# jurihock/sdft

Hardware: AMD Instinct MI355X
Metric: Msamples/s analysis+synthesis, m=1024 Hann fp64; achieved HBM GB/s vs peak (higher is better)
Workload: dtype f64

## Files before the change

sdft_amd/csrc/sdft_capi.inc:

```

#include "sdft_plan.hpp"

#pragma clang fp contract(off)

#define SDFT_CAT_(a, b) a##b
#define SDFT_CAT(a, b) SDFT_CAT_(a, b)
#define SDFT_FN(name) SDFT_CAT(SDFT_CAT(sdft_hip_, name), SDFT_CAT(_, SDFT_SUFFIX))

namespace {
using plan_t = sdfthip::Plan<SDFT_TD, SDFT_FD>;
using fdx_t = sdfthip::cx<SDFT_FD>;
inline plan_t* P(void* p) { return static_cast<plan_t*>(p); }
inline const plan_t* P(const void* p) { return static_cast<const plan_t*>(p); }
}

extern "C" {

void* SDFT_FN(alloc_batch)(size_t dftsize, int window, double latency, size_t channels)
{
  plan_t* p = new (std::nothrow) plan_t();
  if (!p) { sdfthip::set_error("sdft_alloc", "out of host memory"); return nullptr; }
  if (!p->create(dftsize, window, latency, channels)) { p->destroy(); delete p; return nullptr; }
  return p;
}
// ... 146 lines not shown
  if (!p || !key) return -1;
  plan_t* q = P(p);
  if (!strcmp(key, "async")) { if (!value) (void)q->pipe_join(); q->async = value != 0; }
  else if (!strcmp(key, "pipeline")) { if (!value) (void)q->pipe_join(); q->opt_pipeline = value; }
  else if (!strcmp(key, "carry")) q->carry_mode = (value || (sizeof(SDFT_FD) == 4 && !q->opt_float_parallel)) ? sdfthip::CARRY_EXACT : sdfthip::CARRY_FAST;
  else if (!strcmp(key, "float_carry_parallel"))
  {
    q->opt_float_parallel = value != 0;
    if (sizeof(SDFT_FD) == 4) q->carry_mode = value ? sdfthip::CARRY_FAST : sdfthip::CARRY_EXACT;
  }
  else if (!strcmp(key, "exact_inverse")) q->opt_exact_inverse = value;
  else if (!strcmp(key, "host_copy")) q->io.opt_host_copy = value;
  else if (!strcmp(key, "host_register")) { q->io.opt_host_register = value; if (!value) q->io.forget_host_buffers(); }
  else if (!strcmp(key, "copy_threads")) { if (value != q->io.opt_copy_threads) q->io.pool.stop(); q->io.opt_copy_threads = value; }
  else if (!strcmp(key, "pinned_io")) q->opt_pinned_io = value;
  else if (!strcmp(key, "spin")) q->opt_spin = value;
  else if (!strcmp(key, "profile")) q->profile = (int)value;
  else if (!strcmp(key, "resident")) { if (!value) (void)q->resident_retire(); q->opt_resident = value; }
  else if (!strcmp(key, "chunk")) q->opt_chunk = value;
  else if (!strcmp(key, "segments")) q->opt_segments = value;
  else if (!strcmp(key, "chain")) q->opt_chain = value;
  else if (!strcmp(key, "self_carry")) q->opt_self = value;
  else if (!strcmp(key, "hop_kernel")) q->opt_hop_kernel = value;
  else if (!strcmp(key, "fused_exact")) q->opt_fused_exact = value;
  else if (!strcmp(key, "inverse_rows")) q->opt_inverse_rows = value;
  else if (!strcmp(key, "inverse_tune")) { q->opt_inverse_tune = value; for (auto& t : q->inv_tunes) t.reset_all(); }
  else if (!strcmp(key, "pointers")) q->opt_pointers = value;
  else if (!strcmp(key, "stage_bytes")) q->stage_bytes = value > 0 ? (size_t)value : q->stage_bytes;
#ifdef SDFT_HIP_TEST_HOOKS
  else if (!strcmp(key, "interior")) q->opt_interior = value;
  else if (!strcmp(key, "inverse_verify")) q->opt_inverse_verify = value != 0;
  else if (!strcmp(key, "rows_kernel")) q->opt_rows_kernel = value;
  else if (!strcmp(key, "row_slots_max")) q->opt_row_slots_max = value;
  else if (!strcmp(key, "fft_carry")) q->opt_fft_carry = value;
  else if (!strcmp(key, "fused")) q->opt_fused = value;
  else if (!strcmp(key, "fold")) q->opt_fold = value;
  else if (!strcmp(key, "rows_f32")) q->opt_rows_f32 = value;
  else if (!strcmp(key, "hop_parts")) q->opt_hop_parts = value;
  else if (!strcmp(key, "xcd_map")) q->opt_xcd_map = value;
  else if (!strcmp(key, "chain_block")) q->opt_chain_L = value;
  else if (!strcmp(key, "chain_debug")) q->opt_chain_debug = value;
  else if (!strcmp(key, "relay_waves")) q->opt_relay_waves = value;
  else if (!strcmp(key, "relay_flow")) q->opt_relay_flow = value;
  else if (!strcmp(key, "relay_groups")) q->opt_relay_groups = value;
  else if (!strcmp(key, "inverse_nt")) q->opt_inverse_nt = value;
  else if (!strcmp(key, "inverse_nt_skip_mb")) q->opt_inverse_nt_skip_mb = value;
  else if (!strcmp(key, "inverse_step")) q->opt_inverse_step = value;
  else if (!strcmp(key, "inverse_ordered")) q->opt_inverse_ordered = value;
  else if (!strcmp(key, "host_direct")) q->io.opt_host_direct = value;
  else if (!strcmp(key, "copy_streams")) q->io.opt_copy_streams = value;
  else if (!strcmp(key, "array_group")) q->opt_array_group = value;
  else if (!strcmp(key, "mix_group")) q->opt_mix_group = value;
  else if (!strcmp(key, "mix_block")) q->opt_mix_block = value;
  else if (!strcmp(key, "prefix_cells")) q->opt_prefix_cells = value;
#ifdef SDFT_SELF_STAMPS
  else if (!strcmp(key, "self_stamps")) q->opt_self_stamps = value;
#endif
#endif
  else return -1;
  return 0;
}
long SDFT_FN(get_option)(const void* p, const char* key)
{
  if (!p || !key) return -1;
  const plan_t* q = P(p);
  if (!strcmp(key, "async")) return q->async;
  if (!strcmp(key, "pipeline")) return q->opt_pipeline;
  if (!strcmp(key, "last_pipelined")) return q->last_pipelined;
  if (!strcmp(key, "pipelined_calls")) return (long)q->pipe_calls;
  if (!strcmp(key, "pipelined_ordered")) return (long)q->pipe_ordered;
  if (!strcmp(key, "pipelined_inverse_calls")) return (long)q->inv_calls;
  if (!strcmp(key, "last_inverse_pipelined")) return q->last_inverse_pipelined;
  if (!strcmp(key, "pipeline_streams")) return q->pipe_stream_kind * 10 + q->pipe_stream_attempts;
  if (!strcmp(key, "carry")) return q->carry_mode;
  if (!strcmp(key, "float_carry_parallel")) return q->opt_float_parallel;
  if (!strcmp(key, "ordered_walks")) return q->ordered_walks();
  if (!strcmp(key, "inverse_verify")) return q->opt_inverse_verify;
  if (!strcmp(key, "last_inverse_form")) return q->last_inverse_form;
  if (!strcmp(key, "chunk")) return q->opt_chunk;
  if (!strcmp(key, "interior")) return q->interior_lanes();
  if (!strcmp(key, "tiles")) return q->tiles();
  if (!strcmp(key, "bins_per_lane")) return plan_t::bins_per_lane();
  if (!strcmp(key, "last_chunks")) return q->last_chunks;
  if (!strcmp(key, "last_chunk_len")) return q->last_chunk_len;
  if (!strcmp(key, "cursor")) return (long)q->cursor;
  if (!strcmp(key, "last_kernel")) return q->last_kernel;
  if (!strcmp(key, "rows_kernel")) return q->opt_rows_kernel;
  if (!strcmp(key, "fused")) return q->opt_fused;
  if (!strcmp(key, "last_fused")) return q->last_fused;
  if (!strcmp(key, "last_segments")) return q->last_segments;
  if (!strcmp(key, "last_filterbank_launches")) return q->last_filterbank_launches;
  if (!strcmp(key, "row_slots")) return q->row_slots();
  if (!strcmp(key, "device")) return q->device;
  if (!strcmp(key, "last_chain")) return q->last_chain;
  if (!strcmp(key, "last_fused_exact")) return q->last_fused_exact;
  if (!strcmp(key, "last_fused_fold")) return q->last_fused_fold;
  if (!strcmp(key, "last_process_path")) return q->last_process_path;
  if (!strcmp(key, "fused_exact")) return q->opt_fused_exact;
  if (!strcmp(key, "chain")) return q->opt_chain;
  if (!strcmp(key, "fold")) return q->opt_fold;
  if (!strcmp(key, "last_hop_pipe")) return q->last_hop_pipe;
  if (!strcmp(key, "spin")) return q->opt_spin;
  if (!strcmp(key, "inverse_step")) return q->opt_inverse_step;
  if (!strcmp(key, "inverse_ordered")) return q->opt_inverse_ordered;
  if (!strcmp(key, "inverse_nt_skip_mb")) return q->opt_inverse_nt_skip_mb;
  if (!strcmp(key, "last_inverse_nt")) return q->last_inverse_nt;
  if (!strcmp(key, "last_inverse_skip")) return q->last_inverse_skip;
  if (!strcmp(key, "hop_parts")) return q->opt_hop_parts;
  if (!strcmp(key, "xcd_map")) return q->opt_xcd_map;
  if (!strcmp(key, "inverse_tune")) return q->opt_inverse_tune;
  if (!strcmp(key, "last_inverse_tuned")) return q->last_inverse_tuned;
  if (!strcmp(key, "last_hop_parts")) return q->last_hop_parts;
  if (!strcmp(key, "self_carry")) return q->opt_self;
  if (!strcmp(key, "last_self")) return q->last_self;
  if (!strcmp(key, "last_prefix")) return q->last_prefix;
#ifdef SDFT_HIP_TEST_HOOKS
  if (!strcmp(key, "prefix_cells")) return q->opt_prefix_cells;
#endif
  if (!strcmp(key, "array_group")) return q->array_group();
  if (!strcmp(key, "mix_group")) return q->mix_group_size();
  if (!strcmp(key, "mix_block")) return q->mix_block_size();
  if (!strcmp(key, "host_register")) return q->io.opt_host_register;
  if (!strcmp(key, "host_register_hits")) return q->io.host_reg_hits;
  if (!strcmp(key, "host_copy")) return q->io.opt_host_copy;
  if (!strcmp(key, "copy_threads")) return q->io.opt_copy_threads;
  if (!strcmp(key, "copy_streams")) return q->io.opt_copy_streams;
  if (!strcmp(key, "copy_workers")) return (long)q->io.pool.workers();
  if (!strcmp(key, "host_copies_staged")) return q->io.pin_copies;
  if (!strcmp(key, "host_copy_memcpy_us")) return (long)q->io.pin_us_memcpy;
  if (!strcmp(key, "host_copy_device_us")) return (long)q->io.pin_us_device;
  if (!strcmp(key, "host_register_misses")) return q->io.host_reg_misses;
  if (!strcmp(key, "last_flow")) return q->last_flow;
  if (!strcmp(key, "flag_fallbacks")) return q->flag_fallbacks;
  if (!strcmp(key, "ring_recoveries")) return q->ring_recoveries;
  if (!strcmp(key, "rows_f32")) return q->opt_rows_f32;
  if (!strcmp(key, "last_rows_f32")) return q->last_rows_f32;
  if (!strcmp(key, "resident")) return q->opt_resident;
  if (!strcmp(key, "resident_calls")) return (long)q->res.calls;
  if (!strcmp(key, "resident_launches")) return (long)q->res.launches;
  if (!strcmp(key, "resident_missed")) return (long)q->res.missed;
  if (!strcmp(key, "resident_alive")) return q->res.alive ? 1 : 0;
  if (!strcmp(key, "test_hooks"))
  {
#ifdef SDFT_HIP_TEST_HOOKS
    return 1;
#else
    return 0;
#endif
  }
  return -1;
}
int SDFT_FN(get_profile)(void* p, double* ms, long* calls)
{
  if (!p) return -1;
  plan_t* q = P(p);
  if (!q->synchronize()) return -1;
  for (int s = 0; s < sdfthip::ST_COUNT; ++s)
  {
    if (ms) ms[s] = q->prof_ms[s];
    if (calls) calls[s] = q->prof_calls[s];
    q->prof_ms[s] = 0; q->prof_calls[s] = 0;
  }
  return 0;
}
int SDFT_FN(chain_stats)(void* p, unsigned long long* out32) { return p && P(p)->chain_stats(out32) ? 0 : -1; }
int SDFT_FN(relay_stamps)(void* p, unsigned long long* out, size_t count) { return p && P(p)->relay_stamps(out, count) ? 0 : -1; }
int SDFT_FN(get_state)(void* p, void* acc, void* fid, SDFT_TD* hist, size_t* cursor)
{
  return p && P(p)->get_state(static_cast<fdx_t*>(acc), static_cast<fdx_t*>(fid), hist, cursor) ? 0 : -1;
}
// ... 17 lines not shown
```

sdft_amd/csrc/sdft_forward.hpp:

```cpp

#pragma once

#include "sdft_carry_exact.hpp"

#pragma clang fp contract(off)

namespace sdfthip {

template <typename FD, int WIN> SDFT_D cx<FD> window_tap(cx<FD> m2, cx<FD> m1, cx<FD> c0, cx<FD> p1, cx<FD> p2, FD w)
{
  if constexpr (WIN == WIN_HANN)
  {
    const cx<FD> a = cadd(c0, c0);
    const cx<FD> b = cadd(m1, p1);
    return cscale(csub(a, b), w);
  }
  else if constexpr (WIN == WIN_HAMMING)
  {
    const cx<FD> a = cscale(c0, (FD)(0.54));
    const cx<FD> b = cscale(cadd(m1, p1), (FD)(0.23));
    return cscale(csub(a, b), w);
  }
  else if constexpr (WIN == WIN_BLACKMAN)
  {
// ... 85 lines not shown
  r = block - q * d;
  if (r >= d) { --q; r += d; }
}
template <typename FD> SDFT_D void flow_position(const ForwardArgs<FD>& a, unsigned& chunk, size_t& ch, unsigned block)
{
  unsigned q, r;
  if (a.ready) { uniform_divmod(block, a.ready_channels, a.inv_channels, q, r); chunk = a.chunk0 + q; ch = r; }
  else
  {
    if (a.xcd_map) block = xcd_contiguous(block, a.xcd_map);
    uniform_divmod(block, a.launch_chunks, a.inv_chunks, q, r);
    chunk = a.chunk0 + r; ch = q;
  }
}
template <typename FD> SDFT_D void flow_position(const ForwardArgs<FD>& a, unsigned& chunk, size_t& ch) { flow_position(a, chunk, ch, blockIdx.x); }
constexpr unsigned kFlowPollCap = 1u << 19;
template <typename FD> SDFT_D bool flow_wait(const ForwardArgs<FD>& a, unsigned chunk, size_t ch)
{
  if (!a.ready) return true;
  const unsigned* row = a.ready + (ch * a.chunks + chunk) * (size_t)a.ready_n;
  for (unsigned polls = 0;; ++polls)
  {
    bool ok = true;
    for (unsigned i = threadIdx.x; i < a.ready_n; i += blockDim.x)
      ok = ok && __hip_atomic_load(row + i, __ATOMIC_RELAXED, __HIP_MEMORY_SCOPE_AGENT) == a.ready_seq;
    if (__syncthreads_and(ok ? 1 : 0)) break;
    if (polls > kFlowPollCap)
    {
      if (threadIdx.x == 0 && a.ready_status) __hip_atomic_fetch_add(a.ready_status, 1u, __ATOMIC_RELAXED, __HIP_MEMORY_SCOPE_SYSTEM);
      return false;
    }
    if ((polls & 1023u) == 1023u && a.ready_status)
    {
      const bool gone = threadIdx.x == 0 && __hip_atomic_load(a.ready_status, __ATOMIC_RELAXED, __HIP_MEMORY_SCOPE_SYSTEM) != a.ready_status_seen;
      if (__syncthreads_or(gone ? 1 : 0)) return false;
    }
    __builtin_amdgcn_s_sleep(32);
  }
  __builtin_amdgcn_fence(__ATOMIC_ACQUIRE, "agent");
  asm volatile("s_waitcnt vmcnt(0)" ::: "memory");
  __syncthreads();
  return true;
}

template <typename TD, typename FD> struct SelfArgs
{
  const TD* x;
  size_t x_stride;
  const TD* hist_in;
  TD* hist_out;
  const cx<FD>* acc_in;
  unsigned log2m;
  unsigned lds_deltas;
  const FD* prefix;
#ifdef SDFT_SELF_STAMPS
  unsigned long long* stamps;
#endif
  RadixList rl;
};

template <int CP, int QB, typename TD, typename FD>
SDFT_D void self_fold(const SelfArgs<TD, FD>& sa, cx<FD>* cells, unsigned m, unsigned cursor0, size_t ch, size_t t0)
{
  const TD* xs = sa.x + ch * sa.x_stride;
  const TD* hs = sa.hist_in + ch * (size_t)m;
  const unsigned nthr = blockDim.x;
  const size_t rows = (t0 + m - 1) / m;
  for (unsigned v0 = threadIdx.x; v0 < m; v0 += CP * nthr)
  {
    size_t tv[CP]; FD sum[CP]; TD prev[CP];
#pragma unroll
    for (int c = 0; c < CP; ++c)
    {
      const unsigned v = v0 + (unsigned)c * nthr;
      tv[c] = (size_t)(((v < m ? v : v0) + m - cursor0) % m);
      sum[c] = (FD)0;
      prev[c] = hs[tv[c]];
    }
    for (size_t q = 0; q < rows; q += QB)
    {
      TD cur[CP][QB];
#pragma unroll
      for (int c = 0; c < CP; ++c)
#pragma unroll
        for (int qq = 0; qq < QB; ++qq)
        {
          const size_t t = tv[c] + (q + qq) * (size_t)m;
          cur[c][qq] = xs[t < t0 ? t : t0 - 1];
        }
#pragma unroll
      for (int c = 0; c < CP; ++c)
#pragma unroll
        for (int qq = 0; qq < QB; ++qq)
        {
          const size_t t = tv[c] + (q + qq) * (size_t)m;
          if (t < t0) { const TD dd = cur[c][qq] - prev[c]; sum[c] += (FD)dd; prev[c] = cur[c][qq]; }
        }
    }
#pragma unroll
    for (int c = 0; c < CP; ++c)
    {
      const unsigned v = v0 + (unsigned)c * nthr;
      if (v < m) cells[v] = cmake<FD>(sum[c], (FD)0);
    }
  }
}

template <typename FD>
SDFT_D void lds_fft_dif(cx<FD>* x, unsigned log2m, const cx<FD>* __restrict__ w)
{
  const unsigned m = 1u << log2m;
  unsigned st = 0;
  for (; st + 2 <= log2m; st += 2)
  {
    const unsigned half = m >> (st + 1), quarter = half >> 1;
    for (unsigned i = threadIdx.x; i < (m >> 2); i += blockDim.x)
    {
      const unsigned pos = i & (quarter - 1);
      const unsigned base = ((i - pos) << 2) + pos;
      const cx<FD> a0 = x[base], a1 = x[base + quarter], a2 = x[base + half], a3 = x[base + half + quarter];
      const cx<FD> w1 = w[(size_t)pos << st];
      const cx<FD> w2 = w[(size_t)pos << (st + 1)];
      const cx<FD> b0 = cadd(a0, a2), b2 = cmul(csub(a0, a2), w1);
      const cx<FD> b1 = cadd(a1, a3), tq = cmul(csub(a1, a3), w1);
      const cx<FD> b3 = cmake<FD>(tq.im, -tq.re);
      x[base] = cadd(b0, b1);
      x[base + quarter] = cmul(csub(b0, b1), w2);
      x[base + half] = cadd(b2, b3);
      x[base + half + quarter] = cmul(csub(b2, b3), w2);
    }
    __syncthreads();
  }
  if (st < log2m)
  {
    for (unsigned i = threadIdx.x; i < (m >> 1); i += blockDim.x)
    {
      const cx<FD> p = x[2 * i], q = x[2 * i + 1];
      x[2 * i] = cadd(p, q);
      x[2 * i + 1] = csub(p, q);
    }
    __syncthreads();
  }
}

template <typename FD>
SDFT_D cx<FD>* lds_fft_mixed(cx<FD>* x, unsigned m, const RadixList& rl, const cx<FD>* __restrict__ w)
{
  cx<FD>* y = x + m;
  unsigned ns = 1;
  for (unsigned st = 0; st < rl.count; ++st)
  {
    const unsigned r = rl.r[st];
    const unsigned nr = m / r;
    const unsigned tstep = m / (ns * r);
    const unsigned rstep = nr;
    for (unsigned i = threadIdx.x; i < nr; i += blockDim.x)
    {
      const unsigned k = i % ns;
      cx<FD> v[5];
#pragma unroll
      for (unsigned t = 0; t < 5; ++t)
        if (t < r)
        {
          const cx<FD> in = x[i + t * nr];
          v[t] = t == 0 ? in : cmul(in, w[(size_t)(((unsigned long long)t * k * tstep) % m)]);
        }
      const unsigned base = (i / ns) * ns * r + k;
#pragma unroll
      for (unsigned q = 0; q < 5; ++q)
        if (q < r)
        {
          cx<FD> o = v[0];
#pragma unroll
          for (unsigned t = 1; t < 5; ++t)
            if (t < r) o = cadd(o, cmul(v[t], w[(size_t)(((unsigned long long)q * t * rstep) % m)]));
          y[base + q * ns] = o;
        }
    }
    __syncthreads();
    cx<FD>* tmp = x; x = y; y = tmp;
    ns *= r;
  }
  return x;
}

template <typename TD, typename FD> SDFT_D unsigned self_slot(const SelfArgs<TD, FD>& sa, unsigned k)
{
  return sa.log2m ? (__brev(k) >> (32u - sa.log2m)) : k;
}
template <int CP, int QB, typename TD, typename FD>
SDFT_D cx<FD>* self_carry(const SelfArgs<TD, FD>& sa, const ForwardArgs<FD>& a, cx<FD>* cells, unsigned chunk, size_t ch, size_t t0)
{
  const unsigned m = 2u * a.nbins;
  if (chunk + 1 == a.chunks && sa.hist_out)
  {
    const TD* xv = sa.x + ch * sa.x_stride;
    const TD* hv = sa.hist_in + ch * (size_t)m;
    TD* ho = sa.hist_out + ch * (size_t)m;
    for (size_t i = threadIdx.x; i < m; i += blockDim.x)
    {
      const size_t q = a.n + i;
      ho[i] = (q >= m) ? xv[q - m] : hv[q];
    }
  }
  if (t0 == 0) return nullptr;
#ifdef SDFT_SELF_STAMPS
  const bool st_on = sa.stamps && chunk + 1 == a.chunks && threadIdx.x == 0;
  if (st_on) sa.stamps[1] = __builtin_readcyclecounter();
#endif
  if (sa.prefix)
  {
    const FD* pc = sa.prefix + (ch * a.chunks + chunk) * (size_t)m;
    for (unsigned v = threadIdx.x; v < m; v += blockDim.x) cells[v] = cmake<FD>(pc[v], (FD)0);
  }
  else self_fold<CP, QB>(sa, cells, m, a.cursor0, ch, t0);
  __syncthreads();
#ifdef SDFT_SELF_STAMPS
  if (st_on) sa.stamps[2] = __builtin_readcyclecounter();
#endif
  if (sa.log2m)
  {
    lds_fft_dif(cells, sa.log2m, a.wtab);
#ifdef SDFT_SELF_STAMPS
    if (st_on) sa.stamps[3] = __builtin_readcyclecounter();
#endif
    return cells;
  }
  return lds_fft_mixed(cells, m, sa.rl, a.wtab);
}

template <int G, typename TD, typename FD>
SDFT_D void self_deltas(FD (&dl)[G], const SDFT_CONSTANT TD* xs, const SDFT_CONSTANT TD* hs, size_t tt, size_t span)
{
  TD cur[G], old[G];
#pragma unroll
  for (int u = 0; u < G; ++u) cur[u] = xs[tt + u];
  if (tt + G <= span)
  {
#pragma unroll
    for (int u = 0; u < G; ++u) old[u] = hs[tt + u];
  }
  else if (tt >= span)
  {
#pragma unroll
    for (int u = 0; u < G; ++u) old[u] = xs[tt - span + u];
  }
  else
  {
#pragma unroll
    for (int u = 0; u < G; ++u) old[u] = (tt + u < span) ? hs[tt + u] : xs[tt + u - span];
  }
#pragma unroll
  for (int u = 0; u < G; ++u) { const TD dd = cur[u] - old[u]; dl[u] = (FD)dd; }
}
template <typename TD, typename FD>
SDFT_D FD self_delta1(const SDFT_CONSTANT TD* xs, const SDFT_CONSTANT TD* hs, size_t tt, size_t span)
{
  const TD cur = xs[tt];
  const TD old = (tt < span) ? hs[tt] : xs[tt - span];
  const TD dd = cur - old;
  return (FD)dd;
}

typedef double sdft_v2f64 __attribute__((ext_vector_type(2)));
typedef float sdft_v4f32 __attribute__((ext_vector_type(4)));
typedef float sdft_v2f32 __attribute__((ext_vector_type(2)));
template <typename FD, int BPL> struct StoreVec;
template <> struct StoreVec<double, 1> { using type = sdft_v2f64; };
template <> struct StoreVec<float, 2>  { using type = sdft_v4f32; };
template <> struct StoreVec<float, 1>  { using type = sdft_v2f32; };

template <typename V> SDFT_D void store_vec(V* p, V v) { *p = v; }

template <typename FD, int BPL, int WIN, bool ROWS>
__global__ __launch_bounds__(kBlock) void forward_kernel(ForwardArgs<FD> a)
// ... 166 lines not shown
```

sdft_amd/csrc/sdft_forward_rows.hpp:

```cpp

#pragma once

#include "sdft_ops.hpp"

#pragma clang fp contract(off)

namespace sdfthip {

constexpr int kRowWavesMax = 16;
#ifndef SDFT_ROW_GROUP
#define SDFT_ROW_GROUP 8
#endif
#ifndef SDFT_SYN_GROUP_S2F
#define SDFT_SYN_GROUP_S2F 2
#endif
constexpr int kRowGroup = SDFT_ROW_GROUP;

constexpr int kRowSlotsMax = 2;
#ifndef SDFT_SYN_GROUP_S2D
#define SDFT_SYN_GROUP_S2D 4
#endif
#ifndef SDFT_SYN_GROUP_TREE
#define SDFT_SYN_GROUP_TREE 8
#endif
constexpr int syn_group(int S, int BPL, int SYN)
{
  return (S == 2 && BPL == 2 && SYN == 1) ? SDFT_SYN_GROUP_S2F : (SYN == 1 && S == 1) ? SDFT_SYN_GROUP_TREE
       : (S == 2 && BPL == 1) ? SDFT_SYN_GROUP_S2D : kRowGroup / S;
}

template <typename FD, int BPL, int WIN, bool FUSED, int S, int SYN = 0, bool LAT1 = true, typename TD = float, bool SELF = false>
__global__ __launch_bounds__(kWave * kRowWavesMax) void forward_rows_kernel(ForwardArgs<FD> a, FuseArgs<TD, FD> fz, SelfArgs<TD, FD> sa)
{
  static_assert(!SELF || SYN == 0, "the self-carried form shares the dynamic LDS with the terms image");
  constexpr int H = win_halo<WIN>::value;
  constexpr int G = SYN != 0 ? syn_group(S, BPL, SYN) : ((kRowGroup / (S * BPL)) >= 2 ? kRowGroup / (S * BPL) : 2);
  constexpr int HS = 2;
  constexpr int VW = kRowWavesMax * S;
  __shared__ cx<FD> edgeL[2][G][VW][HS];
  __shared__ cx<FD> edgeR[2][G][VW][HS];
  extern __shared__ __align__(16) unsigned char rows_dyn_lds[];
  FD* terms = reinterpret_cast<FD*>(rows_dyn_lds);

  const int lane = threadIdx.x & (kWave - 1);
  const int wave = __builtin_amdgcn_readfirstlane(threadIdx.x >> 6);
  const int nwaves = blockDim.x >> 6;
  const int nv = nwaves * S;
  unsigned chunk; size_t ch;
  flow_position(a, chunk, ch);
#ifdef SDFT_SELF_STAMPS
  if constexpr (SELF) { if (sa.stamps && chunk + 1 == a.chunks && threadIdx.x == 0) sa.stamps[0] = __builtin_readcyclecounter(); }
#endif
  if (!flow_wait(a, chunk, ch)) return;

  const long nbins = (long)a.nbins;
  const unsigned span = 2u * a.nbins, maxc = span - 1u;
  const size_t t0 = chunk ? (size_t)chunk * a.chunk_len - a.chunk_shift : 0;
  const size_t tn = (size_t)(chunk + 1) * a.chunk_len - a.chunk_shift;
  const size_t t1 = tn < a.n ? tn : a.n;
  unsigned c = (unsigned)(((size_t)a.cursor0 + t0) % span);

  cx<FD>* cells = reinterpret_cast<cx<FD>*>(rows_dyn_lds);
  cx<FD>* dft = nullptr;
  if constexpr (SELF) dft = self_carry<2, (sizeof(TD) == 8 ? 8 : 16)>(sa, a, cells, chunk, ch, t0);

  const long vlast_bin = (long)nv * kWave * BPL - 1;
  BinState<FD> s[S][BPL];
  bool keep[S][BPL], flip[S][BPL];
  cx<FD>* pub[S][BPL];
  bool pubflip[S][BPL], has_role[S][BPL];
  unsigned flipmask[S][BPL], pubmask[S][BPL];
  const size_t cbase = (ch * a.chunks + chunk) * a.nbins;
#pragma unroll
  for (int q = 0; q < S; ++q)
  {
    const int v = q * nwaves + wave;
    const long wfirst = (long)v * kWave * BPL;
    const long wlast = wfirst + (long)kWave * BPL - 1;
#pragma unroll
    for (int b = 0; b < BPL; ++b)
    {
      const long k = wfirst + (long)lane * BPL + b;
      const long kk = reflect_bin(k, nbins, flip[q][b]);
      keep[q][b] = k < nbins;
      s[q][b].tw = a.tw[kk];
      if constexpr (SELF)
      {
        s[q][b].acc = sa.acc_in[ch * a.nbins + kk];
        if (dft) s[q][b].acc = cadd(s[q][b].acc, dft[self_slot(sa, (unsigned)kk)]);
        s[q][b].fid = a.wtab[((unsigned)kk * c) % span];
      }
      else
      {
      s[q][b].acc = a.carry[cbase + kk];
      s[q][b].fid = a.fseed ? fid_from_table(a.fseed, a.fseed_L, a.nbins, kk, c, s[q][b].tw)
                  : a.seed  ? a.seed[cbase + kk] : a.wtab[((unsigned)kk * c) % span];
      }

      pub[q][b] = &edgeL[0][0][0][0];
      pubflip[q][b] = false; has_role[q][b] = false;
      if (H >= 1)
      {
#pragma unroll
        for (int i = 0; i < HS; ++i)
        {
          if (v + 1 < nv && k == wlast - i) { pub[q][b] = &edgeL[0][0][v + 1][i]; has_role[q][b] = true; }
          if (v > 0 && k == wfirst + i) { pub[q][b] = &edgeR[0][0][v - 1][i]; has_role[q][b] = true; }
        }
#pragma unroll
        for (int i = 0; i < HS; ++i)
        {
          bool f0; const long r0 = reflect_bin(-1 - i, nbins, f0);
          if (k == r0) { pub[q][b] = &edgeL[0][0][0][i]; pubflip[q][b] = f0; has_role[q][b] = true; }
          if (vlast_bin - (nbins - 1) < H)
          {
            bool f1; const long r1 = reflect_bin(vlast_bin + 1 + i, nbins, f1);
            if (k == r1) { pub[q][b] = &edgeR[0][0][nv - 1][i]; pubflip[q][b] = f1; has_role[q][b] = true; }
          }
        }
      }
    }
  }
#pragma unroll
  for (int q = 0; q < S; ++q)
#pragma unroll
    for (int b = 0; b < BPL; ++b)
    {
      flipmask[q][b] = flip[q][b] ? 0x80000000u : 0u;
      pubmask[q][b] = (flip[q][b] != pubflip[q][b]) ? 0x80000000u : 0u;
    }
  constexpr size_t kSlabU = (size_t)VW * HS;
  constexpr size_t kSlabBuf = (size_t)G * kSlabU;

  const SDFT_CONSTANT FD* d = as_uniform(a.delta + ch * a.n);
  const SDFT_CONSTANT TD* xin = SELF ? as_uniform(sa.x + ch * sa.x_stride) : nullptr;
  const SDFT_CONSTANT TD* hin = SELF ? as_uniform(sa.hist_in + ch * (size_t)span) : nullptr;
  const FD w = a.wscale;
  cx<FD>* row = a.out + ch * a.out_stride + t0 * (size_t)a.nbins;
  unsigned off_elems[S];
#pragma unroll
  for (int q = 0; q < S; ++q)
  {
    off_elems[q] = (unsigned)(((q * nwaves + wave) * kWave + lane) * BPL);
    __builtin_assume(off_elems[q] < (1u << 20));
  }

// ... 343 lines not shown
```

sdft_amd/csrc/sdft_plan.hpp:

```cpp

#pragma once

#include "sdft_kernels.hpp"
#include "sdft_forward_rows_f32.hpp"
#include "sdft_resident.hpp"
#include "sdft_plan_logic.hpp"
#include "sdft_host_io.hpp"

#include <limits.h>
#include <math.h>
#include <stdio.h>
#include <stdlib.h>
#include <string.h>

#include <algorithm>
#if defined(__SSE2__)
#include <emmintrin.h>
#endif
#include <chrono>
#include <string>
#include <vector>

#pragma clang fp contract(off)

// ... 99 lines not shown
#endif
  long opt_inverse_verify = 1, last_inverse_form = 0;
  bool rtc_failed = false;
  std::string user_expr;
  template <typename T> static const char* type_name() { return sizeof(T) == 8 ? "double" : "float"; }
  long opt_float_parallel = 0;
  long opt_chunk = 0;
  long opt_interior = 0;
  size_t stage_bytes = logic::kDefaultStageBytes;
  int profile = 0;
  long opt_rows_kernel = 1;
  long opt_xcd_map = 1;
  long opt_pinned_io = 1;
  long opt_pointers = 0;
  long opt_inverse_rows = 0;
  size_t inverse_capacity[2] = {0, 0};
  long opt_inverse_nt = -1;
  long opt_inverse_nt_skip_mb = -1;
  long opt_inverse_tune = 1, last_inverse_tuned = 0;
  logic::TunerTable inv_tunes[2];
  bool inv_after_write = false;
  hipEvent_t tune_evs[2][logic::TunerTable::kSlots][logic::FormTuner::kMax][2] = {};
  bool ensure_tune_events()
  {
    if (tune_evs[0][0][0][0]) return true;
    for (auto& kind : tune_evs)
      for (auto& tuner : kind)
        for (auto& pair : tuner)
          for (hipEvent_t& e : pair)
            if (hipEventCreate(&e) != hipSuccess)
            {
              (void)hipGetLastError(); e = nullptr;
              destroy_tune_events();
              return false;
            }
    return true;
  }
  void destroy_tune_events()
  {
    for (auto& kind : tune_evs) for (auto& tuner : kind) for (auto& q : tuner) for (hipEvent_t& f : q) if (f) { (void)hipEventDestroy(f); f = nullptr; }
  }
  long opt_exact_inverse = 1;
  long opt_row_slots_max = 2;
  long opt_fused = 1;
  long last_fused = 0;
  long opt_fft_carry = 1;
  long opt_hop_kernel = 1;
  long opt_fused_exact = -1;
  long last_fused_exact = 0, last_fused_fold = 0, last_process_path = 0;
  long opt_spin = 1;
  long opt_self = 1;
  long last_self = 0;
  long opt_prefix_cells = 1;
  long last_prefix = 0;

  long last_kernel = 0;

  DevBuf<fdx> d_tw, d_syn, d_wtab;
  DevBuf<fdx> d_accs[4], d_fids[4];
  int st_cur = 0;
  fdx* acc_p() { return d_accs[st_cur].p; }
  fdx* fid_p() { return d_fids[st_cur].p; }
  DevBuf<TD> d_hist[4];
  int hist_cur = 0;
  size_t cursor = 0;

  hipStream_t aux = nullptr;
  std::vector<hipEvent_t> seg_events;
  hipEvent_t ev_delta = nullptr;
  DevBuf<fdx> d_run_acc[2], d_run_fid[2];
  long opt_segments = 0;
  long last_segments = 1;

  DevBuf<fdx> d_fseed;
  unsigned fseed_L = 0;
  bool fid_canonical = true;
  long opt_chain = 1;
  long opt_chain_L = 0, opt_chain_debug = 0;
  long last_hop_pipe = 0;
  long opt_hop_parts = 0, last_hop_parts = 1;
  long opt_fold = 1;
  long opt_relay_waves = 0;
  DevBuf<unsigned long long> d_chain_stats;
  long last_chain = 0;

  DevBuf<FD> d_delta;
  DevBuf<fdx> d_carry, d_seed;
  DevBuf<FD> d_prefix;
  DevBuf<TD> d_stage_td;
  DevBuf<fdx> d_stage_fdx;
  DevBuf<fdx*> d_rowptr;
  DevBuf<FD> d_psum_ws, d_psum_head;
  struct Filterbank
  {
    std::vector<size_t> bin0, nbins;
    std::vector<FD> weights;
    logic::FilterbankLayout layout;
    long interior = -1;
  } fbank;
  DevBuf<FilterbankPiece> d_fb_pieces;
  DevBuf<unsigned> d_fb_tile0;
  DevBuf<FilterbankSplit> d_fb_splits;
  DevBuf<FD> d_fb_weights, d_fb_ws;
  struct Pairs
  {
    std::vector<size_t> a, b;
// ... 737 lines not shown
      if (inv.used[i]) { SDFT_TRY(hipStreamWaitEvent(stream, ev_inv[i], 0)); inv.used[i] = false; }
    return true;
  }
  bool pipe_join() { return pipe_join_rows() && pipe_join_inverses(); }
  bool pipe_join_rows()
  {
    if (!ring.open) return true;
    int slots[2];
    const int count = ring.last_per_stream(slots);
    for (int i = 0; i < count; ++i) SDFT_TRY(hipStreamWaitEvent(stream, ev_rows[slots[i]], 0));
    ring.joined();
    return true;
  }
  void release_pipe()
  {
    for (int i = 0; i < 2; ++i) if (row_streams[i]) { (void)hipStreamSynchronize(row_streams[i]); (void)hipStreamDestroy(row_streams[i]); row_streams[i] = nullptr; }
    if (ev_pre) { (void)hipEventDestroy(ev_pre); ev_pre = nullptr; }
    for (int i = 0; i < 4; ++i) if (ev_rows[i]) { (void)hipEventDestroy(ev_rows[i]); ev_rows[i] = nullptr; }
    for (int i = 0; i < 2; ++i) { if (ev_inv[i]) { (void)hipEventDestroy(ev_inv[i]); ev_inv[i] = nullptr; } inv.used[i] = false; }
    ring.joined();
    (void)hipGetLastError();
  }
  bool pipe_wanted(const void* fuse) const
  {
    return !fuse && pipe_allowed && async && own_stream && !stream_exposed && opt_pipeline && profile == 0 && sizeof(FD) == 8;
  }
  bool launch_self_state(const ForwardArgs<FD>& fa, const SelfArgs<TD, FD>& sa, unsigned threads)
  {
    auto kern = self_state_kernel<TD, FD>;
    const size_t lds = self_cells() * sizeof(fdx);
    static thread_local int raised_on = -1;
    if (raised_on != device)
    {
      SDFT_TRY(hipFuncSetAttribute(reinterpret_cast<const void*>(kern), hipFuncAttributeMaxDynamicSharedMemorySize, (int)(96 * 1024)));
      raised_on = device;
    }
    hipLaunchKernelGGL(kern, dim3((unsigned)channels), dim3(threads), lds, stream, fa, sa);
    SDFT_TRY(hipGetLastError());
    return true;
  }

  bool forward_self(size_t n, const TD* x, size_t x_stride, fdx* out, size_t out_stride, long chunks, long len,
                    const FuseArgs<TD, FD>* fuse, bool prefix = false)
  {
    const size_t nb = nbins, span = 2 * nbins;
    SelfArgs<TD, FD> sa;
    sa.x = x; sa.x_stride = x_stride;
    sa.hist_in = d_hist[hist_cur].p; sa.hist_out = d_hist[hist_cur ^ 1].p;
    sa.acc_in = d_accs[st_cur].p;
    sa.log2m = 0; sa.rl.count = 0;
    if ((span & (span - 1)) == 0) while (((size_t)1 << sa.log2m) < span) ++sa.log2m;
    else sa.rl = smooth_radices(span);
    sa.lds_deltas = 0;
    sa.prefix = nullptr;
#ifdef SDFT_SELF_STAMPS
    sa.stamps = reinterpret_cast<unsigned long long*>(opt_self_stamps);
#endif
    ForwardArgs<FD> fa{};
    fa.delta = nullptr; fa.tw = d_tw.p; fa.wtab = d_wtab.p; fa.carry = nullptr; fa.seed = nullptr; fa.fseed = nullptr; fa.fseed_L = 0;
    fa.out = out; fa.out_stride = out_stride; fa.out_rows = nullptr;
    fa.acc_state = d_accs[st_cur ^ 1].p; fa.fid_state = d_fids[st_cur ^ 1].p; fa.n = n;
    fa.total_waves = 0;
    fa.nbins = (unsigned)nb; fa.chunks = (unsigned)chunks; fa.chunk_len = (unsigned)len; fa.tiles = (unsigned)tiles();
    fa.interior_lanes = (unsigned)interior_lanes(); fa.cursor0 = (unsigned)cursor; fa.chunk_shift = 0;
    fa.chunk0 = 0; fa.launch_chunks = (unsigned)chunks; fa.inv_chunks = inv32(fa.launch_chunks);
    fa.xcd_map = logic::xcd_groups(opt_xcd_map != 0, channels * (size_t)chunks);
    fa.vec_store = 0;
    fa.wscale = (window == WIN_HANN) ? (FD)(tab.aweight * (FD)(0.25)) : tab.aweight;
    fa.done.flag = nullptr; fa.done.count = nullptr; fa.done.seq = 0; fa.done.total = 0;
    if (!grid_fits(channels * (size_t)chunks)) return false;
    if (channels * n * nb <= (fuse ? logic::kFlagMaxFused : logic::kFlagMax)) fa.done = arm_flag((unsigned)(channels * (size_t)chunks));
    const unsigned blocks = (unsigned)(channels * (size_t)chunks);
    const bool fused = opt_fused != 0;
    last_fused = fused; last_segments = 1; last_chain = 0;
    last_pipelined = 0;
    if constexpr (sizeof(FD) == 8)
    {
      const uintptr_t olo = reinterpret_cast<uintptr_t>(out), ohi = olo + ((channels - 1) * out_stride + n * nb) * sizeof(fdx);
      if (pipe_this && !fuse && ensure_pipe())
      {
        if (!pipe_join_inverses()) return false;
        const uintptr_t xlo = reinterpret_cast<uintptr_t>(x), xhi = xlo + ((channels - 1) * x_stride + n) * sizeof(TD);
        if (ring.samples_overlap(xlo, xhi) && !pipe_join()) return false;
        const int s1 = (st_cur + 1) & 3, h1 = (hist_cur + 1) & 3;
        const logic::RowRing::Pick pk = ring.pick(olo, ohi);
        const int rsi = pk.stream;
        hipStream_t rs = row_streams[rsi];
        SDFT_TRY(hipEventRecord(ev_pre, stream));
        SDFT_TRY(hipStreamWaitEvent(rs, ev_pre, 0));
        if (pk.behind)
        {
          ++pipe_ordered;
          if (pk.wait_launch >= 0) SDFT_TRY(hipStreamWaitEvent(rs, ev_rows[pk.wait_launch], 0));
        }
        if (ring.state_reader() >= 0) SDFT_TRY(hipStreamWaitEvent(stream, ev_rows[ring.state_reader()], 0));
        ForwardArgs<FD> fs = fa; SelfArgs<TD, FD> ss = sa;
        fs.acc_state = d_accs[s1].p; fs.fid_state = d_fids[s1].p; ss.hist_out = d_hist[h1].p;
        fs.done.flag = nullptr; fs.done.count = nullptr; fs.done.seq = 0; fs.done.total = 0;
        if (!launch_self_state(fs, ss, (unsigned)(row_waves() * kWave))) return false;
        ForwardArgs<FD> fr = fa; SelfArgs<TD, FD> sr = sa;
        fr.acc_state = nullptr; fr.fid_state = nullptr; sr.hist_out = nullptr;
        fr.done.flag = nullptr; fr.done.count = nullptr; fr.done.seq = 0; fr.done.total = 0;
        {
          Scoped<hipStream_t> on(stream, rs);
          if (!launch_forward_rows_self(fr, sr, blocks, (unsigned)(row_waves() * kWave), fused)) return false;
        }
// ... 398 lines not shown
```

Before: 419.6.

## Hoist self-carry prologue loads ahead of fold and FFT, use buffer loads

Restructures the self-carry prologue of the forward rows kernel. Per-bin state loads (twiddle, accumulator, fid), the history delay-line read and the first-stage FFT twiddles are issued before the fold and FFT, so their latency overlaps that work instead of following it. The fold now uses raw buffer loads with a split between full rows and a remainder, which removes the per-element bounds check and the 64-bit modulo. The previous path is kept behind test hooks. In exchange, more values stay live in registers across the fold and FFT, which may reduce occupancy.

```diff
diff --git a/sdft_amd/csrc/sdft_capi.inc b/sdft_amd/csrc/sdft_capi.inc
--- a/sdft_amd/csrc/sdft_capi.inc
+++ b/sdft_amd/csrc/sdft_capi.inc
@@ -222,6 +222,7 @@
   else if (!strcmp(key, "array_group")) q->opt_array_group = value;
   else if (!strcmp(key, "mix_group")) q->opt_mix_group = value;
   else if (!strcmp(key, "mix_block")) q->opt_mix_block = value;
+  else if (!strcmp(key, "self_prologue")) q->opt_self_prologue = value;
   else if (!strcmp(key, "prefix_cells")) q->opt_prefix_cells = value;
 #ifdef SDFT_SELF_STAMPS
   else if (!strcmp(key, "self_stamps")) q->opt_self_stamps = value;
@@ -286,6 +287,7 @@
   if (!strcmp(key, "last_prefix")) return q->last_prefix;
 #ifdef SDFT_HIP_TEST_HOOKS
   if (!strcmp(key, "prefix_cells")) return q->opt_prefix_cells;
+  if (!strcmp(key, "self_prologue")) return q->opt_self_prologue;
 #endif
   if (!strcmp(key, "array_group")) return q->array_group();
   if (!strcmp(key, "mix_group")) return q->mix_group_size();
diff --git a/sdft_amd/csrc/sdft_forward.hpp b/sdft_amd/csrc/sdft_forward.hpp
--- a/sdft_amd/csrc/sdft_forward.hpp
+++ b/sdft_amd/csrc/sdft_forward.hpp
@@ -161,6 +161,7 @@
   const cx<FD>* acc_in;
   unsigned log2m;
   unsigned lds_deltas;
+  unsigned parent_prologue;
   const FD* prefix;
 #ifdef SDFT_SELF_STAMPS
   unsigned long long* stamps;
@@ -168,8 +169,123 @@
   RadixList rl;
 };
 
+template <typename TD, typename FD> SDFT_D bool self_parent_prologue(const SelfArgs<TD, FD>& sa)
+{
+#ifdef SDFT_HIP_TEST_HOOKS
+  return sa.parent_prologue != 0;
+#else
+  (void)sa;
+  return false;
+#endif
+}
+
+template <typename TD> SDFT_D __amdgpu_buffer_rsrc_t fold_rows(const TD* base, unsigned bytes)
+{
+  return __builtin_amdgcn_make_buffer_rsrc(const_cast<TD*>(base), 0, (int)bytes, 0x00020000);
+}
+template <typename TD> SDFT_D TD fold_load(__amdgpu_buffer_rsrc_t rows, unsigned lane_bytes, unsigned row_bytes)
+{
+  if constexpr (sizeof(TD) == 4) return __builtin_bit_cast(TD, __builtin_amdgcn_raw_buffer_load_b32(rows, (int)lane_bytes, (int)row_bytes, 0));
+  else return __builtin_bit_cast(TD, __builtin_amdgcn_raw_buffer_load_b64(rows, (int)lane_bytes, (int)row_bytes, 0));
+}
+
+template <int I> struct RowTag { static constexpr int value = I; };
+template <int I, int N, typename F> SDFT_D void first_rows(unsigned count, F&& f)
+{
+  if constexpr (I < N)
+  {
+    if ((unsigned)I < count) { f(RowTag<I>{}); first_rows<I + 1, N>(count, f); }
+  }
+}
+
 template <int CP, int QB, typename TD, typename FD>
 SDFT_D void self_fold(const SelfArgs<TD, FD>& sa, cx<FD>* cells, unsigned m, unsigned cursor0, size_t ch, size_t t0)
+{
+  const TD* xs = sa.x + ch * sa.x_stride;
+  const TD* hs = sa.hist_in + ch * (size_t)m;
+  const unsigned nthr = blockDim.x;
+  const size_t full = sa.log2m ? t0 >> sa.log2m : t0 / m;
+  const unsigned rem = (unsigned)(t0 - full * m);
+  const unsigned row_bytes = m * (unsigned)sizeof(TD);
+  for (unsigned v0 = threadIdx.x; v0 < m; v0 += CP * nthr)
+  {
+    unsigned tv[CP]; FD sum[CP]; TD prev[CP];
+#pragma unroll
+    for (int c = 0; c < CP; ++c)
+    {
+      const unsigned v = v0 + (unsigned)c * nthr;
+      const unsigned u = (v < m ? v : v0) + m - cursor0;
+      tv[c] = u >= m ? u - m : u;
+      sum[c] = (FD)0;
+      prev[c] = hs[tv[c]];
+    }
+    const TD* rp = xs;
+    size_t q = 0;
+    for (; q + QB <= full; q += QB, rp += (size_t)QB * m)
+    {
+      const __amdgpu_buffer_rsrc_t rows = fold_rows(rp, (unsigned)QB * row_bytes);
+      TD cur[CP][QB];
+#pragma unroll
+      for (int c = 0; c < CP; ++c)
+#pragma unroll
+        for (int qq = 0; qq < QB; ++qq) cur[c][qq] = fold_load<TD>(rows, tv[c] * (unsigned)sizeof(TD), (unsigned)qq * row_bytes);
+#pragma unroll
+      for (int c = 0; c < CP; ++c)
+#pragma unroll
+        for (int qq = 0; qq < QB; ++qq)
+        {
+          const TD dd = cur[c][qq] - prev[c];
+          sum[c] += (FD)dd; prev[c] = cur[c][qq];
+        }
+    }
+    const unsigned left = (unsigned)(full - q);
+    if (left != 0 || rem != 0)
+    {
+      const __amdgpu_buffer_rsrc_t rows = fold_rows(rp, left * row_bytes + rem * (unsigned)sizeof(TD));
+      TD cur[CP][QB], cut[CP];
+      first_rows<0, QB - 1>(left, [&](auto row)
+      {
+        constexpr int qq = decltype(row)::value;
+#pragma unroll
+        for (int c = 0; c < CP; ++c) cur[c][qq] = fold_load<TD>(rows, tv[c] * (unsigned)sizeof(TD), (unsigned)qq * row_bytes);
+      });
+#pragma unroll
+      for (int c = 0; c < CP; ++c)
+      {
+        cut[c] = (TD)0;
+        if (tv[c] < rem) cut[c] = fold_load<TD>(rows, tv[c] * (unsigned)sizeof(TD), left * row_bytes);
+      }
+      asm volatile("" ::: "memory");
+      first_rows<0, QB - 1>(left, [&](auto row)
+      {
+        constexpr int qq = decltype(row)::value;
+#pragma unroll
+        for (int c = 0; c < CP; ++c)
+        {
+          const TD dd = cur[c][qq] - prev[c];
+          sum[c] += (FD)dd; prev[c] = cur[c][qq];
+        }
+      });
+#pragma unroll
+      for (int c = 0; c < CP; ++c)
+        if (tv[c] < rem)
+        {
+          const TD dd = cut[c] - prev[c];
+          sum[c] += (FD)dd; prev[c] = cut[c];
+        }
+    }
+#pragma unroll
+    for (int c = 0; c < CP; ++c)
+    {
+      const unsigned v = v0 + (unsigned)c * nthr;
+      if (v < m) cells[v] = cmake<FD>(sum[c], (FD)0);
+    }
+  }
+}
+
+#ifdef SDFT_HIP_TEST_HOOKS
+template <int CP, int QB, typename TD, typename FD>
+SDFT_D void self_fold_parent(const SelfArgs<TD, FD>& sa, cx<FD>* cells, unsigned m, unsigned cursor0, size_t ch, size_t t0)
 {
   const TD* xs = sa.x + ch * sa.x_stride;
   const TD* hs = sa.hist_in + ch * (size_t)m;
@@ -216,7 +332,7 @@
 }
 
 template <typename FD>
-SDFT_D void lds_fft_dif(cx<FD>* x, unsigned log2m, const cx<FD>* __restrict__ w)
+SDFT_D void lds_fft_dif_parent(cx<FD>* x, unsigned log2m, const cx<FD>* __restrict__ w)
 {
   const unsigned m = 1u << log2m;
   unsigned st = 0;
@@ -251,6 +367,67 @@
     __syncthreads();
   }
 }
+#endif
+
+template <typename FD>
+SDFT_D void lds_fft_twiddles(cx<FD>& w1, cx<FD>& w2, unsigned log2m, unsigned st, const cx<FD>* __restrict__ w)
+{
+  const unsigned quarter = (1u << log2m) >> (st + 2);
+  if (threadIdx.x < (1u << (log2m - 2)))
+  {
+    const unsigned pos = threadIdx.x & (quarter - 1);
+    w1 = w[(size_t)pos << st];
+    w2 = w[(size_t)pos << (st + 1)];
+  }
+}
+
+template <typename FD>
+SDFT_D void lds_fft_dif(cx<FD>* x, unsigned log2m, const cx<FD>* __restrict__ w, cx<FD> w1, cx<FD> w2)
+{
+  const unsigned m = 1u << log2m;
+  unsigned st = 0;
+  for (; st + 2 <= log2m; st += 2)
+  {
+    const unsigned half = m >> (st + 1), quarter = half >> 1;
+    cx<FD> n1 = w1, n2 = w2;
+    if (st + 4 <= log2m) lds_fft_twiddles(n1, n2, log2m, st + 2, w);
+    auto butterfly = [&](unsigned i, cx<FD> u1, cx<FD> u2)
+    {
+      const unsigned pos = i & (quarter - 1);
+      const unsigned base = ((i - pos) << 2) + pos;
+      const cx<FD> a0 = x[base], a1 = x[base + quarter], a2 = x[base + half], a3 = x[base + half + quarter];
+      const cx<FD> b0 = cadd(a0, a2), b2 = cmul(csub(a0, a2), u1);
+      const cx<FD> b1 = cadd(a1, a3), tq = cmul(csub(a1, a3), u1);
+      const cx<FD> b3 = cmake<FD>(tq.im, -tq.re);
+      x[base] = cadd(b0, b1);
+      x[base + quarter] = cmul(csub(b0, b1), u2);
+      x[base + half] = cadd(b2, b3);
+      x[base + half + quarter] = cmul(csub(b2, b3), u2);
+    };
+    unsigned i = threadIdx.x;
+    if (i < (m >> 2))
+    {
+      butterfly(i, w1, w2);
+      for (i += blockDim.x; i < (m >> 2); i += blockDim.x)
+      {
+        const unsigned pos = i & (quarter - 1);
+        butterfly(i, w[(size_t)pos << st], w[(size_t)pos << (st + 1)]);
+      }
+    }
+    __syncthreads();
+    w1 = n1; w2 = n2;
+  }
+  if (st < log2m)
+  {
+    for (unsigned i = threadIdx.x; i < (m >> 1); i += blockDim.x)
+    {
+      const cx<FD> p = x[2 * i], q = x[2 * i + 1];
+      x[2 * i] = cadd(p, q);
+      x[2 * i + 1] = csub(p, q);
+    }
+    __syncthreads();
+  }
+}
 
 template <typename FD>
 SDFT_D cx<FD>* lds_fft_mixed(cx<FD>* x, unsigned m, const RadixList& rl, const cx<FD>* __restrict__ w)
@@ -297,8 +474,9 @@
 {
   return sa.log2m ? (__brev(k) >> (32u - sa.log2m)) : k;
 }
+#ifdef SDFT_HIP_TEST_HOOKS
 template <int CP, int QB, typename TD, typename FD>
-SDFT_D cx<FD>* self_carry(const SelfArgs<TD, FD>& sa, const ForwardArgs<FD>& a, cx<FD>* cells, unsigned chunk, size_t ch, size_t t0)
+SDFT_D cx<FD>* self_carry_parent(const SelfArgs<TD, FD>& sa, const ForwardArgs<FD>& a, cx<FD>* cells, unsigned chunk, size_t ch, size_t t0)
 {
   const unsigned m = 2u * a.nbins;
   if (chunk + 1 == a.chunks && sa.hist_out)
@@ -322,14 +500,92 @@
     const FD* pc = sa.prefix + (ch * a.chunks + chunk) * (size_t)m;
     for (unsigned v = threadIdx.x; v < m; v += blockDim.x) cells[v] = cmake<FD>(pc[v], (FD)0);
   }
-  else self_fold<CP, QB>(sa, cells, m, a.cursor0, ch, t0);
+  else self_fold_parent<CP, QB>(sa, cells, m, a.cursor0, ch, t0);
   __syncthreads();
 #ifdef SDFT_SELF_STAMPS
   if (st_on) sa.stamps[2] = __builtin_readcyclecounter();
 #endif
   if (sa.log2m)
   {
-    lds_fft_dif(cells, sa.log2m, a.wtab);
+    lds_fft_dif_parent(cells, sa.log2m, a.wtab);
+#ifdef SDFT_SELF_STAMPS
+    if (st_on) sa.stamps[3] = __builtin_readcyclecounter();
+#endif
+    return cells;
+  }
+  return lds_fft_mixed(cells, m, sa.rl, a.wtab);
+}
+#endif
+
+constexpr int kLineRegs = 4;
+template <typename TD, typename FD> struct DelayLine
+{
+  const TD* from_x; const TD* from_h; TD* to;
+  unsigned m, old;
+  bool on;
+  TD held[kLineRegs];
+  SDFT_D TD source(unsigned i) const { return i < old ? from_h[i] : from_x[i - old]; }
+  SDFT_D void request(const SelfArgs<TD, FD>& sa, const ForwardArgs<FD>& a, unsigned chunk, size_t ch)
+  {
+    m = 2u * a.nbins;
+    on = chunk + 1 == a.chunks && sa.hist_out;
+    if (!on) return;
+    to = sa.hist_out + ch * (size_t)m;
+    const TD* xv = sa.x + ch * sa.x_stride;
+    const TD* hv = sa.hist_in + ch * (size_t)m;
+    if (a.n >= m) { old = 0; from_h = hv; from_x = xv + (a.n - m); }
+    else { old = m - (unsigned)a.n; from_h = hv + a.n; from_x = xv; }
+#pragma unroll
+    for (int j = 0; j < kLineRegs; ++j)
+    {
+      const unsigned i = threadIdx.x + (unsigned)j * blockDim.x;
+      held[j] = (TD)0;
+      if (i < m) held[j] = source(i);
+    }
+  }
+  SDFT_D void store() const
+  {
+    if (!on) return;
+#pragma unroll
+    for (int j = 0; j < kLineRegs; ++j)
+    {
+      const unsigned i = threadIdx.x + (unsigned)j * blockDim.x;
+      if (i < m) to[i] = held[j];
+    }
+    for (unsigned i = threadIdx.x + (unsigned)kLineRegs * blockDim.x; i < m; i += blockDim.x) to[i] = source(i);
+  }
+};
+
+template <int CP, int QB, typename TD, typename FD>
+SDFT_D cx<FD>* self_carry(const SelfArgs<TD, FD>& sa, const ForwardArgs<FD>& a, cx<FD>* cells, unsigned chunk, size_t ch, size_t t0)
+{
+#ifdef SDFT_HIP_TEST_HOOKS
+  if (self_parent_prologue(sa)) return self_carry_parent<CP, QB>(sa, a, cells, chunk, ch, t0);
+#endif
+  const unsigned m = 2u * a.nbins;
+  DelayLine<TD, FD> line;
+  line.request(sa, a, chunk, ch);
+  if (t0 == 0) { line.store(); return nullptr; }
+#ifdef SDFT_SELF_STAMPS
+  const bool st_on = sa.stamps && chunk + 1 == a.chunks && threadIdx.x == 0;
+  if (st_on) sa.stamps[1] = __builtin_readcyclecounter();
+#endif
+  cx<FD> w1 = cmake<FD>((FD)0, (FD)0), w2 = w1;
+  if (sa.log2m >= 2) lds_fft_twiddles(w1, w2, sa.log2m, 0, a.wtab);
+  if (sa.prefix)
+  {
+    const FD* pc = sa.prefix + (ch * a.chunks + chunk) * (size_t)m;
+    for (unsigned v = threadIdx.x; v < m; v += blockDim.x) cells[v] = cmake<FD>(pc[v], (FD)0);
+  }
+  else self_fold<CP, QB>(sa, cells, m, a.cursor0, ch, t0);
+  line.store();
+  __syncthreads();
+#ifdef SDFT_SELF_STAMPS
+  if (st_on) sa.stamps[2] = __builtin_readcyclecounter();
+#endif
+  if (sa.log2m)
+  {
+    lds_fft_dif(cells, sa.log2m, a.wtab, w1, w2);
 #ifdef SDFT_SELF_STAMPS
     if (st_on) sa.stamps[3] = __builtin_readcyclecounter();
 #endif
diff --git a/sdft_amd/csrc/sdft_forward_rows.hpp b/sdft_amd/csrc/sdft_forward_rows.hpp
--- a/sdft_amd/csrc/sdft_forward_rows.hpp
+++ b/sdft_amd/csrc/sdft_forward_rows.hpp
@@ -58,14 +58,36 @@
   const size_t t0 = chunk ? (size_t)chunk * a.chunk_len - a.chunk_shift : 0;
   const size_t tn = (size_t)(chunk + 1) * a.chunk_len - a.chunk_shift;
   const size_t t1 = tn < a.n ? tn : a.n;
-  unsigned c = (unsigned)(((size_t)a.cursor0 + t0) % span);
+  unsigned c;
+  if (SELF && sa.log2m) c = ((unsigned)t0 + a.cursor0) & maxc;
+  else c = (unsigned)(((size_t)a.cursor0 + t0) % span);
 
   cx<FD>* cells = reinterpret_cast<cx<FD>*>(rows_dyn_lds);
   cx<FD>* dft = nullptr;
-  if constexpr (SELF) dft = self_carry<2, (sizeof(TD) == 8 ? 8 : 16)>(sa, a, cells, chunk, ch, t0);
+  BinState<FD> s[S][BPL];
+  auto self_state = [&]()
+  {
+#pragma unroll
+    for (int q = 0; q < S; ++q)
+#pragma unroll
+      for (int b = 0; b < BPL; ++b)
+      {
+        bool f;
+        const long kk = reflect_bin((long)(q * nwaves + wave) * kWave * BPL + (long)lane * BPL + b, (long)a.nbins, f);
+        s[q][b].tw = a.tw[kk];
+        s[q][b].acc = sa.acc_in[ch * a.nbins + kk];
+        s[q][b].fid = a.wtab[((unsigned)kk * c) % span];
+      }
+  };
+  (void)self_state;
+  if constexpr (SELF)
+  {
+    if (!self_parent_prologue(sa)) self_state();
+    dft = self_carry<2, (sizeof(TD) == 8 ? 8 : 16)>(sa, a, cells, chunk, ch, t0);
+    if (self_parent_prologue(sa)) self_state();
+  }
 
   const long vlast_bin = (long)nv * kWave * BPL - 1;
-  BinState<FD> s[S][BPL];
   bool keep[S][BPL], flip[S][BPL];
   cx<FD>* pub[S][BPL];
   bool pubflip[S][BPL], has_role[S][BPL];
@@ -83,15 +105,13 @@
       const long k = wfirst + (long)lane * BPL + b;
       const long kk = reflect_bin(k, nbins, flip[q][b]);
       keep[q][b] = k < nbins;
+      if constexpr (SELF)
+      {
+        if (dft) s[q][b].acc = cadd(s[q][b].acc, dft[self_slot(sa, (unsigned)kk)]);
+      }
+      else
+      {
       s[q][b].tw = a.tw[kk];
-      if constexpr (SELF)
-      {
-        s[q][b].acc = sa.acc_in[ch * a.nbins + kk];
-        if (dft) s[q][b].acc = cadd(s[q][b].acc, dft[self_slot(sa, (unsigned)kk)]);
-        s[q][b].fid = a.wtab[((unsigned)kk * c) % span];
-      }
-      else
-      {
       s[q][b].acc = a.carry[cbase + kk];
       s[q][b].fid = a.fseed ? fid_from_table(a.fseed, a.fseed_L, a.nbins, kk, c, s[q][b].tw)
                   : a.seed  ? a.seed[cbase + kk] : a.wtab[((unsigned)kk * c) % span];
diff --git a/sdft_amd/csrc/sdft_plan.hpp b/sdft_amd/csrc/sdft_plan.hpp
--- a/sdft_amd/csrc/sdft_plan.hpp
+++ b/sdft_amd/csrc/sdft_plan.hpp
@@ -175,6 +175,7 @@
   long opt_self = 1;
   long last_self = 0;
   long opt_prefix_cells = 1;
+  long opt_self_prologue = 1;
   long last_prefix = 0;
 
   long last_kernel = 0;
@@ -1018,6 +1019,10 @@
     if ((span & (span - 1)) == 0) while (((size_t)1 << sa.log2m) < span) ++sa.log2m;
     else sa.rl = smooth_radices(span);
     sa.lds_deltas = 0;
+    sa.parent_prologue = 0;
+#ifdef SDFT_HIP_TEST_HOOKS
+    sa.parent_prologue = opt_self_prologue ? 0u : 1u;
+#endif
     sa.prefix = nullptr;
 #ifdef SDFT_SELF_STAMPS
     sa.stamps = reinterpret_cast<unsigned long long*>(opt_self_stamps);
```

Measured after the change: 421.7 (median of 2 runs). Within noise of the previous version (+0.5%).
